# mmaker/c-lwe-snarks

Measured on AMD Instinct MI355X. Metric: snark_proofs_per_sec, higher is better.
Workload: dtype u32 limbs (704-bit integers mod 2^704) + AES-256 bytes; int8 digits on the matrix cores, int32 accumulation (exact)

## Files before the change

c-lwe-snarks_amd/csrc/ctx.hpp:

```cpp
#pragma once
#include <hip/hip_runtime.h>

#include <stdint.h>
#include <string.h>

#include <string>
#include <vector>

#include "aes_dev.hpp"
#include "mfhip.h"
#include "ssp_prg.hpp"

#define HIP_TRY(ctx, expr)                                                        \
  do {                                                                            \
    hipError_t e_ = (expr);                                                       \
    if (e_ != hipSuccess) {                                                       \
      (ctx)->err = std::string(#expr) + ": " + hipGetErrorString(e_);             \
      return MFH_EDEVICE;                                                         \
    }                                                                             \
  } while (0)

struct PolyState;
struct SspInterp;
struct SspRows;
// ... 262 lines not shown
  uint64_t cstride;
  uint32_t bits_row0;
  const uint64_t *add_ct;
  const uint32_t *add_scale;
  uint32_t sa_from1;
};
int eval_rows_multi_io(mfh_ctx *c, uint64_t off, size_t nrows, const uint8_t *d_c8, const MmIo &io, uint32_t nvec, uint32_t coeff_bytes, int accumulate);
int eval_rows_multi_io_set(mfh_ctx *c, uint64_t off, size_t nrows, const uint8_t *d_c8, const MmIo *ios, const uint32_t *nvecs, uint32_t ng,
                           uint32_t coeff_bytes);
struct MmRegion { uint64_t off; const uint8_t *c8; };
int eval_rows_multi_io_regions(mfh_ctx *c, const MmRegion *regs, uint32_t nreg, size_t nrows, const MmIo *ios, const uint32_t *nvecs, uint32_t ng,
                               uint32_t coeff_bytes, int accumulate);
bool mm_image_covers(const mfh_ctx *c, uint64_t off, size_t nrows);
struct MmsPlan {
  uint32_t ng, ngt, ND, nrows, nchunks, rpc, rpad, ntiles, mtiles;
  size_t cd_bytes, part_bytes;
  const uint8_t *img[2];
  int8_t *cd;
  int *part;
};
bool mms_plan(mfh_ctx *c, const MmRegion *regs, uint32_t nreg, size_t nrows, const MmIo *ios, const uint32_t *nvecs, uint32_t ng, uint32_t coeff_bytes,
              MmsPlan &P);
size_t mms_ws_bytes(const MmsPlan &P);
void mms_bind(MmsPlan &P, void *ws);
int mms_digits(mfh_ctx *c, const MmsPlan &P, const MmIo *ios, const uint32_t *nvecs);
int mms_stream(mfh_ctx *c, const MmsPlan &P);
int mms_finish(mfh_ctx *c, const MmsPlan &P, const MmIo *ios, const uint32_t *nvecs, int accumulate);
```

c-lwe-snarks_amd/csrc/evalmm.hip:

```cpp
#include <algorithm>
#include <cstring>

#include "ctx.hpp"

namespace {

using mf::AesKey;

constexpr int CT = 4;
constexpr int SB = 88;
constexpr int VB = 92;
constexpr int MB = CT * SB;
constexpr int MT = MB / 32;
constexpr int RT = 128;
constexpr int TSTRIDE = 384;
constexpr int BLK_PER_ROW = 24;
static_assert(MB % 32 == 0 && CT * VB + 15 <= TSTRIDE, "tile geometry");

typedef int v4i __attribute__((ext_vector_type(4)));
typedef int v16i __attribute__((ext_vector_type(16)));

__device__ __forceinline__ uint32_t coef_at(const MmIo &io, uint32_t v, uint32_t nrows, uint32_t i) {
  if (io.bits) {
    const uint32_t a = io.bits_row0 + i;
// ... 467 lines not shown
constexpr int CH = NQ2 / CG;
struct MmsImages { const v4i *image[16]; };
__device__ __forceinline__ void mms_item(uint32_t xcd, uint32_t slot, uint32_t ngt, uint32_t ngr, uint32_t map, uint32_t &grp, uint32_t &tg) {
  if (map == 0) {
    grp = slot % ngt;
    tg = (slot / ngt) * 8 + xcd;
  } else {
    const uint32_t blk = slot >> 5, i = slot & 31, nreg = ngt / ngr, tpb = 32 / ngr;
    grp = (blk % nreg) * ngr + i % ngr;
    tg = ((blk / nreg) * tpb + i / ngr) * 8 + xcd;
  }
}
__device__ __forceinline__ long long mms_pack_e(const v4i &a) {
  return (long long)a[0] + ((long long)a[1] << 8) + ((long long)a[2] << 16) + ((long long)a[3] << 24);
}
template <int CTRL>
__device__ __forceinline__ long long mms_quad_bcast(long long t) {
  const int lo = __builtin_amdgcn_update_dpp(0, (int)(unsigned int)(unsigned long long)t, CTRL, 0xf, 0xf, false);
  const int hi = __builtin_amdgcn_update_dpp(0, (int)((unsigned long long)t >> 32), CTRL, 0xf, 0xf, false);
  return (long long)(((unsigned long long)(unsigned int)hi << 32) | (unsigned int)lo);
}
__device__ __forceinline__ void mms_store_packed(int *__restrict__ part, uint32_t pk, uint64_t m4 , uint32_t ctile, uint32_t c16,
                                                 const v4i &acc) {
  const long long T = mms_pack_e(acc);
  if (pk == 1) {
    reinterpret_cast<long long *>(part)[m4 * N2 + 16 * ctile + c16] = T;
    return;
  }
  const long long T1 = mms_quad_bcast<0x55>(T), T2 = mms_quad_bcast<0xAA>(T), T3 = mms_quad_bcast<0xFF>(T);
  if (c16 & 3) return;
  const __int128 U = (__int128)T + (__int128)T1 * 256 + (__int128)T2 * 65536 + (__int128)T3 * 16777216;
  const unsigned __int128 u = (unsigned __int128)U;
  reinterpret_cast<uint4 *>(part)[m4 * (N2 / 4) + 4 * ctile + (c16 >> 2)] = uint4{(uint32_t)u, (uint32_t)(u >> 32), (uint32_t)(u >> 64), 0u};
}
__device__ __forceinline__ void mmstream_body(const MmsImages &imgs, uint32_t mtiles, uint32_t KS, uint32_t nrows, uint32_t rows_per_chunk,
                                              const v4i *__restrict__ cdv, int *__restrict__ part, uint32_t grp, uint32_t tg ,
                                              uint32_t chunk, uint64_t cd_stride , uint64_t part_stride , uint32_t pk ) {
  __shared__ v4i bfrag[2][RT2 / 64][NQ2][64];
  const uint32_t tid = threadIdx.x, lane = tid & 63;
  const uint32_t wave = __builtin_amdgcn_readfirstlane(tid >> 6);
  const uint32_t c16 = lane & 15, g4 = lane >> 4;
  const uint32_t rq = wave % RG, ch = wave / RG;
  if (tg * 16 >= mtiles) return;
  const v4i *__restrict__ image = imgs.image[grp];
  cdv += grp * cd_stride;
  part += grp * part_stride;
  const uint32_t mt0 = (tg * RG + rq) * RQ;
  const uint32_t r0 = chunk * rows_per_chunk, r1 = min(nrows, r0 + rows_per_chunk);
  v4i acc[RQ][CH];
#pragma unroll
  for (int t = 0; t < RQ; t++)
#pragma unroll
    for (int q = 0; q < CH; q++) acc[t][q] = v4i{0, 0, 0, 0};
// ... 70 lines not shown
#pragma unroll
      for (int t = 0; t < RQ; t++) a[t][ks] = a_load(t, un1, ks);
#pragma unroll
      for (int i = 0; i < BPK; i++) bnr[ks][i] = b_load(un2, ks, i);
    }
#ifndef MMS_NOSYNC
    __syncthreads();
#endif
    buf ^= 1;
  }
  const uint64_t Mtot = (uint64_t)mtiles * 16;
#ifdef MMS_ACC_ASM
  asm volatile("s_nop 15\n\ts_nop 15" ::: "memory");
#endif
  if (pk) {
#pragma unroll
    for (int t = 0; t < RQ; t++) {
      if (mt0 + t >= mtiles) continue;
      const uint64_t m4 = (uint64_t)chunk * (Mtot / 4) + (uint64_t)(mt0 + t) * 4 + g4;
#pragma unroll
      for (int q = 0; q < CH; q++) mms_store_packed(part, pk, m4, ch * CH + q, c16, acc[t][q]);
    }
    return;
  }
#pragma unroll
  for (int t = 0; t < RQ; t++) {
    if (mt0 + t >= mtiles) continue;
    int *p = part + ((uint64_t)chunk * Mtot + (uint64_t)(mt0 + t) * 16) * N2;
#pragma unroll
    for (int q = 0; q < CH; q++)
#pragma unroll
      for (int e = 0; e < 4; e++) p[(uint64_t)(4 * g4 + e) * N2 + 16 * (ch * CH + q) + c16] = acc[t][q][e];
  }
}

__global__ __launch_bounds__(SW * 64) void k_mmstream(MmsImages imgs, uint32_t mtiles, uint32_t KS, uint32_t nrows, uint32_t rows_per_chunk,
                                                      const v4i *__restrict__ cdv, int *__restrict__ part, uint32_t ngt, uint32_t ngr, uint32_t map,
                                                      uint64_t cd_stride, uint64_t part_stride, uint32_t pk) {
  uint32_t grp, tg;
  mms_item(blockIdx.x & 7, blockIdx.x >> 3, ngt, ngr, map, grp, tg);
  mmstream_body(imgs, mtiles, KS, nrows, rows_per_chunk, cdv, part, grp, tg, blockIdx.y, cd_stride, part_stride, pk);
}
__global__ __launch_bounds__(SW * 64) void k_mmstream1(MmsImages imgs, uint32_t mtiles, uint32_t KS, uint32_t nrows, uint32_t rows_per_chunk,
                                                       const v4i *__restrict__ cdv, int *__restrict__ part, uint32_t pk) {
  mmstream_body(imgs, mtiles, KS, nrows, rows_per_chunk, cdv, part, 0u, blockIdx.x, blockIdx.y, 0, 0, pk);
}
__device__ __forceinline__ void mmstream_persistent(const MmsImages &imgs, uint32_t mtiles, uint32_t KS, uint32_t nrows, uint32_t rows_per_chunk,
                                                    const v4i *__restrict__ cdv, int *__restrict__ part, uint32_t ngt, uint32_t ngr, uint32_t map,
                                                    uint64_t cd_stride, uint64_t part_stride, uint32_t nblk , uint32_t nchunks,
                                                    uint32_t *__restrict__ sync, uint32_t sync_mode, uint32_t spin_max, uint32_t width, uint32_t pk) {
  const uint32_t xcd = blockIdx.x & 7, cu = blockIdx.x >> 3;
  const uint32_t members = sync_mode == 2 ? 32u : (map ? ngr : ngt);
  uint32_t *ctr = sync + xcd * 32 + (sync_mode == 2 ? 0u : cu / members);
  uint32_t k = 0;
  for (uint32_t chunk = 0; chunk < nchunks; chunk++)
    for (uint32_t slot = cu; slot < nblk * 32; slot += width, k++) {
      if (sync_mode && members > 1) {
        if (threadIdx.x == 0) {
          __hip_atomic_fetch_add(ctr, 1u, __ATOMIC_RELAXED, __HIP_MEMORY_SCOPE_AGENT);
          const uint32_t target = (k + 1) * members;
          for (uint32_t spin = 0; spin < spin_max && __hip_atomic_load(ctr, __ATOMIC_RELAXED, __HIP_MEMORY_SCOPE_AGENT) < target; spin++) __builtin_amdgcn_s_sleep(8);
        }
        __syncthreads();
      }
      uint32_t grp, tg;
      mms_item(xcd, slot, ngt, ngr, map, grp, tg);
      mmstream_body(imgs, mtiles, KS, nrows, rows_per_chunk, cdv, part, grp, tg, chunk, cd_stride, part_stride, pk);
    }
}
__global__ __launch_bounds__(SW * 64) void k_mmstream_p(MmsImages imgs, uint32_t mtiles, uint32_t KS, uint32_t nrows, uint32_t rows_per_chunk,
                                                        const v4i *__restrict__ cdv, int *__restrict__ part, uint32_t ngt, uint32_t ngr, uint32_t map,
                                                        uint64_t cd_stride, uint64_t part_stride, uint32_t nblk, uint32_t nchunks,
                                                        uint32_t *__restrict__ sync, uint32_t sync_mode, uint32_t spin_max, uint32_t width, uint32_t pk) {
  mmstream_persistent(imgs, mtiles, KS, nrows, rows_per_chunk, cdv, part, ngt, ngr, map, cd_stride, part_stride, nblk, nchunks, sync, sync_mode, spin_max, width, pk);
}
__global__ __launch_bounds__(SW * 64) void k_mmstream_pb(MmsImages imgs, uint32_t mtiles, uint32_t KS, uint32_t nrows, uint32_t rows_per_chunk,
                                                         const v4i *__restrict__ cdv, int *__restrict__ part, uint32_t ngt, uint32_t ngr, uint32_t map,
                                                         uint64_t cd_stride, uint64_t part_stride, uint32_t nblk, uint32_t nchunks,
                                                         uint32_t *__restrict__ sync, uint32_t sync_mode, uint32_t spin_max, uint32_t width, uint32_t pk) {
  mmstream_persistent(imgs, mtiles, KS, nrows, rows_per_chunk, cdv, part, ngt, ngr, map, cd_stride, part_stride, nblk, nchunks, sync, sync_mode, spin_max, width, pk);
}

constexpr int WSW = 4, WRQ = 4;
__device__ __forceinline__ void mfma_acc(v4i &acc, const v4i &a, const v4i &b) {
  asm volatile("v_mfma_i32_16x16x64_i8 %0, %1, %2, %0" : "+a"(acc) : "v"(a), "v"(b));
}
__device__ __forceinline__ void mmstream_body_w(const MmsImages &imgs, uint32_t mtiles, uint32_t KS, uint32_t nrows, uint32_t rows_per_chunk,
                                                const v4i *__restrict__ cdv, int *__restrict__ part, uint32_t grp, uint32_t tg, uint32_t chunk, uint64_t cd_stride,
                                                uint64_t part_stride) {
  __shared__ v4i bfrag[2][RT2 / 64][NQ2][64];
  const uint32_t tid = threadIdx.x, lane = tid & 63;
  const uint32_t wave = __builtin_amdgcn_readfirstlane(tid >> 6);
  const uint32_t c16 = lane & 15, g4 = lane >> 4;
  if (tg * 16 >= mtiles) return;
  const v4i *__restrict__ image = imgs.image[grp];
// ... 90 lines not shown
                                                         const v4i *__restrict__ cdv, int *__restrict__ part, uint32_t ngt, uint32_t ngr, uint32_t map,
                                                         uint64_t cd_stride, uint64_t part_stride, uint32_t nblk, uint32_t nchunks) {
  const uint32_t xcd = blockIdx.x & 7, cu = blockIdx.x >> 3;
  for (uint32_t k = 0; k < nblk * nchunks; k++) {
    uint32_t grp, tg;
    mms_item(xcd, (k % nblk) * 32 + cu, ngt, ngr, map, grp, tg);
    mmstream_body_w(imgs, mtiles, KS, nrows, rows_per_chunk, cdv, part, grp, tg, k / nblk, cd_stride, part_stride);
  }
}

template <int ND, int KWM ,
          bool PK >
__device__ __forceinline__ void evalmm_finish_body(const int *__restrict__ part, const int64_t *__restrict__ sc, uint32_t nchunks, uint32_t ntiles, uint32_t N,
                                                   uint32_t nvec, uint32_t n, uint32_t nrows, uint32_t ct, uint32_t MBv, uint32_t sby, uint32_t LL,
                                                   const MmIo &io, int accumulate, const int *__restrict__ sa_part, uint32_t sa_col) {
  __shared__ uint32_t sv[KWM][3][64];
  const uint32_t vl = threadIdx.x & 63, lq = threadIdx.x >> 6;
  const uint32_t v = blockIdx.y * 64 + vl, j = blockIdx.x;
  const uint32_t tile = j / ct, jj = j % ct;
  const uint32_t KWv = sby / 4;
  if (v < nvec) {
    int64_t corr[ND];
#pragma unroll
    for (int w = 0; w < ND; w++) corr[w] = 128 * sc[ND * v + w] + 16384ll * nrows;
    if (PK) {
      const uint64_t M4 = (uint64_t)ntiles * MBv / 4;
      unsigned __int128 corrsum = 0;
#pragma unroll
      for (int w = 0; w < ND; w++) corrsum += (unsigned __int128)((uint64_t)corr[w] * 0x01010101ull) << (8 * w);
      for (uint32_t l = lq; l < KWv; l += 4) {
        const uint64_t m4 = ((uint64_t)tile * MBv + jj * sby) / 4 + l;
        __int128 U = 0, SA = 0;
        for (uint32_t ch = 0; ch < nchunks; ch++) {
          const uint64_t at = (uint64_t)ch * M4 + m4;
          if (ND == 4) {
            const uint4 r = reinterpret_cast<const uint4 *>(part)[at * (N / 4) + v], q = reinterpret_cast<const uint4 *>(sa_part)[at * (N / 4) + sa_col / 4];
            U += (__int128)(((unsigned __int128)(uint64_t)(int64_t)(int32_t)r.z << 64) | ((uint64_t)r.y << 32) | r.x);
            SA += (__int128)(((unsigned __int128)(uint64_t)(int64_t)(int32_t)q.z << 64) | ((uint64_t)q.y << 32) | q.x);
          } else {
            U += reinterpret_cast<const long long *>(part)[at * N + v];
            SA += reinterpret_cast<const long long *>(sa_part)[at * N + sa_col];
          }
        }
        const unsigned __int128 val = (unsigned __int128)(U + SA * (__int128)(ND == 4 ? 128ll * 0x01010101ll : 128ll)) + corrsum;
        sv[l][0][vl] = (uint32_t)val;
        sv[l][1][vl] = (uint32_t)(val >> 32);
        sv[l][2][vl] = (uint32_t)(val >> 64);
      }
    } else
    for (uint32_t l = lq; l < KWv; l += 4) {
      unsigned __int128 val = 0;
      int g0[4][ND], sa0[4];
#pragma unroll
      for (int k = 0; k < 4; k++) {
        const int *row = part + ((uint64_t)tile * MBv + (jj * sby + 4 * l + k)) * N;
#pragma unroll
        for (int w = 0; w < ND; w++) g0[k][w] = row[ND * v + w];
        sa0[k] = (sa_part + ((uint64_t)tile * MBv + (jj * sby + 4 * l + k)) * N)[sa_col];
      }
#pragma unroll
      for (int k = 0; k < 4; k++) {
        const uint32_t mm = jj * sby + 4 * l + k;
        int64_t g[ND], sa = sa0[k];
#pragma unroll
        for (int w = 0; w < ND; w++) g[w] = g0[k][w];
        for (uint32_t ch = 1; ch < nchunks; ch++) {
          const int *row = part + (((uint64_t)ch * ntiles + tile) * MBv + mm) * N;
#pragma unroll
          for (int w = 0; w < ND; w++) g[w] += row[ND * v + w];
          sa += (sa_part + (((uint64_t)ch * ntiles + tile) * MBv + mm) * N)[sa_col];
        }
        uint64_t t = 0;
#pragma unroll
        for (int w = 0; w < ND; w++) t += (uint64_t)(g[w] + 128 * sa + corr[w]) << (8 * w);
        val += (unsigned __int128)t << (8 * k);
      }
      sv[l][0][vl] = (uint32_t)val;
      sv[l][1][vl] = (uint32_t)(val >> 32);
      sv[l][2][vl] = (uint32_t)(val >> 64);
    }
  }
  __syncthreads();
  if (lq != 0 || v >= nvec) return;
  uint32_t *out = reinterpret_cast<uint32_t *>((v < io.osplit ? io.out[0] + (uint64_t)v * io.ostride : io.out[1] + (uint64_t)(v - io.osplit) * io.ostride) +
                                               (uint64_t)j * LL);
  const bool wide4 = (LL & 1) == 0 && (io.ostride & 1) == 0 && ((reinterpret_cast<uintptr_t>(io.out[0]) | reinterpret_cast<uintptr_t>(io.out[1])) & 15) == 0;
  uint32_t pend[4] = {0, 0, 0, 0};
  uint64_t carry = 0;
  const uint32_t *actw = io.add_ct ? reinterpret_cast<const uint32_t *>(io.add_ct + (uint64_t)j * LL) : nullptr;
  const uint64_t ax = io.add_ct ? io.add_scale[v] : 0;
  uint64_t acarry = 0;
  for (uint32_t l = 0; l < KWv; l++) {
    uint64_t word = carry + sv[l][0][vl];
    if (l >= 1) word += sv[l - 1][1][vl];
    if (l >= 2) word += sv[l - 2][2][vl];
    if (accumulate) word += out[l];
    if (actw) {
      const uint64_t t = (uint64_t)actw[l] * ax + acarry;
      word += (uint32_t)t;
      acarry = t >> 32;
    }
    carry = word >> 32;
    pend[l & 3] = (uint32_t)word;
    if (wide4 ? (l & 3) == 3 : (l & 1) == 1) {
      if (wide4) *reinterpret_cast<uint4 *>(out + (l & ~3u)) = uint4{pend[0], pend[1], pend[2], pend[3]};
      else *reinterpret_cast<uint2 *>(out + (l & ~1u)) = uint2{pend[(l & 2)], pend[(l & 2) + 1]};
    }
  }
  if (wide4) {
    if (KWv & 3) *reinterpret_cast<uint4 *>(out + (KWv & ~3u)) = uint4{pend[0], (KWv & 3) > 1 ? pend[1] : 0u, (KWv & 3) > 2 ? pend[2] : 0u, 0u};
// ... 16 lines not shown
                                                               int accumulate) {
  const uint32_t g = blockIdx.z, lender = A.io[g].sa_from1 ? A.io[g].sa_from1 - 1 : g;
  evalmm_finish_body<ND, KWM, PK>(part + g * part_stride, A.io[g].sc_zeroed, nchunks, ntiles, N, A.nvec[g], n, nrows, ct, MBv, sby, LL, A.io[g], accumulate,
                                  part + lender * part_stride, ND * A.nvec[lender]);
}

}

extern "C" {

struct WideGeom { uint32_t ct, sby, vby, mt, mbp, LL; };
static WideGeom wide_geom(const mfh_ctx *c) {
  if (c->P.logq == 736) return {W16<736>::CT, W16<736>::SBY, W16<736>::VBY, W16<736>::MT, W16<736>::MBP, W16<736>::LL};
  return {W16<1472>::CT, W16<1472>::SBY, W16<1472>::VBY, W16<1472>::MT, W16<1472>::MBP, W16<1472>::LL};
}

#define FINISH_LAUNCH(kern, ND_, PK_, grid, ...)                                                                         \
  do {                                                                                                                   \
    if ((PK_) && wg.sby / 4 <= 22) hipLaunchKernelGGL((kern<ND_, 22, true>), grid, dim3(256), 0, c->stream, __VA_ARGS__);  \
    else if (PK_) hipLaunchKernelGGL((kern<ND_, 46, true>), grid, dim3(256), 0, c->stream, __VA_ARGS__);                 \
    else if (wg.sby / 4 <= 22) hipLaunchKernelGGL((kern<ND_, 22, false>), grid, dim3(256), 0, c->stream, __VA_ARGS__);   \
    else hipLaunchKernelGGL((kern<ND_, 46, false>), grid, dim3(256), 0, c->stream, __VA_ARGS__);                         \
  } while (0)

int mfh_eval_rows_multi(mfh_ctx *c, uint64_t off, size_t nrows, const uint8_t *d_c8, const uint32_t *d_coeffs, uint32_t nvec, uint32_t coeff_bytes,
                        uint64_t *d_rops, int accumulate) {
  if (!c || !d_rops || !nvec || (nrows && (!d_c8 || !d_coeffs)) || (coeff_bytes != 1 && coeff_bytes != 4)) return MFH_EINVAL;
  const MmIo io = {{d_coeffs, nullptr}, nvec, {d_rops, nullptr}, nvec, (uint64_t)(c->P.n + 1) * wide_geom(c).LL, nullptr, 0, nullptr};
  return eval_rows_multi_io(c, off, nrows, d_c8, io, nvec, coeff_bytes, accumulate);
}
// ... 29 lines not shown
    }
    return MFH_OK;
  }
  const uint32_t ct = wide ? wg.ct : CT, mb = wide ? wg.mbp : CT * SB, rt = wide ? RT2 : RT;
  const uint32_t NT = wide ? NQ2 : (nvec * ND + 1 <= 64 ? 2 : 4), N = wide ? N2 : 32 * NT;
  const uint32_t ntiles = (n + 1 + ct - 1) / ct;
  uint32_t nchunks = (!wide && nrows >= 8 * rt) ? 2 : 1;
  const uint32_t lim = std::max(rt, c->mm_chunk_rows / rt * rt);
  nchunks = std::max<uint32_t>(nchunks, ((uint32_t)nrows + lim - 1) / lim);
  uint32_t rpc = ((uint32_t)nrows + nchunks - 1) / nchunks;
  rpc = (rpc + rt - 1) / rt * rt;
  nchunks = ((uint32_t)nrows + rpc - 1) / rpc;
  const uint32_t rpad = nchunks * rpc;
  const size_t cd_bytes = ((size_t)N * rpad + 255) & ~(size_t)255;
  const size_t sc_bytes = 256 * 8;
  const size_t part_bytes = (size_t)nchunks * ntiles * mb * N * 4;
  int rc = c->mm_ws_sel ? ws2_reserve(c, cd_bytes + sc_bytes + part_bytes) : ws_reserve(c, cd_bytes + sc_bytes + part_bytes);
  if (rc) return rc;
  uint8_t *wsp = (c->mm_ws_sel ? c->ws2 : c->ws).as<uint8_t>();
  int8_t *cd = (int8_t *)wsp;
  int64_t *sc = io.sc_zeroed ? io.sc_zeroed : (int64_t *)(wsp + cd_bytes);
  int *part = (int *)(wsp + cd_bytes + sc_bytes);
  if (!io.sc_zeroed) HIP_TRY(c, hipMemsetAsync(sc, 0, sc_bytes, c->stream));
  if (wide && ND == 4 && !io.bits)
    hipLaunchKernelGGL(k_mm_digits4w, dim3((rpad / 16 + DG4 - 1) / DG4), dim3(256), 0, c->stream, io, nvec, (uint32_t)nrows, rpad, cd, sc);
  else
    hipLaunchKernelGGL(k_mm_digits, dim3((rpad / 16 + DG_RG - 1) / DG_RG), dim3(N), 0, c->stream, io, nvec, ND, (uint32_t)nrows, rpad, NT, wide ? 1 : 0, cd, sc);
  AesKey keyx = c->key;
  for (int i = 56; i < 60; i++) keyx.rk[i] ^= 0x80808080u;
  const uint32_t pk = img_region && c->mm_pack ? ND : 0u;
  {
    Timer t(c, img_region ? 8 : 7, nrows);
    if (img_region) {
      const uint32_t mtiles = ntiles * wg.mt, KS = ((uint32_t)nrows + RT2 - 1) / RT2 * (RT2 / 64);
      MmsImages imgs{};
      imgs.image[0] = (const v4i *)img_region;
      hipLaunchKernelGGL(k_mmstream1, dim3(((mtiles + TPW - 1) / TPW + 7) / 8 * 8, nchunks), dim3(SW * 64), 0, c->stream, imgs,
                         mtiles, KS, (uint32_t)nrows, rpc, (const v4i *)cd, part, pk);
    } else if (wide && q736)
      hipLaunchKernelGGL((k_evalmm16<0, 736>), dim3(ntiles, nchunks), dim3(1024), 0, c->stream, keyx, c->d_t0, off, n, (uint32_t)nrows, rpc, d_c8, cd, part,
                         (uint8_t *)nullptr);
    else if (wide)
      hipLaunchKernelGGL((k_evalmm16<0, 1472>), dim3(ntiles, nchunks), dim3(1024), 0, c->stream, keyx, c->d_t0, off, n, (uint32_t)nrows, rpc, d_c8, cd, part,
                         (uint8_t *)nullptr);
    else if (NT == 2)
      hipLaunchKernelGGL(k_evalmm<2>, dim3(ntiles, nchunks), dim3(1024), 0, c->stream, keyx, c->d_t0, off, n, (uint32_t)nrows, rpc, d_c8, cd, rpad,
                         part);
    else
      hipLaunchKernelGGL(k_evalmm<4>, dim3(ntiles, nchunks), dim3(1024), 0, c->stream, keyx, c->d_t0, off, n, (uint32_t)nrows, rpc, d_c8, cd, rpad,
                         part);
  }
  HIP_TRY(c, hipGetLastError());
  const uint32_t sby = wide ? wg.sby : SB;
  const dim3 fgrid(n + 1, (nvec + 63) / 64);
  if (ND == 4)
    FINISH_LAUNCH(k_evalmm_finish, 4, pk, fgrid, part, sc, nchunks, ntiles, N, nvec, n, (uint32_t)nrows, ct, mb, sby, wg.LL, io, accumulate);
  else
    FINISH_LAUNCH(k_evalmm_finish, 1, pk, fgrid, part, sc, nchunks, ntiles, N, nvec, n, (uint32_t)nrows, ct, mb, sby, wg.LL, io, accumulate);
  HIP_TRY(c, hipGetLastError());
  return MFH_OK;
}

bool mms_plan(mfh_ctx *c, const MmRegion *regs, uint32_t nreg, size_t nrows, const MmIo *ios, const uint32_t *nvecs, uint32_t ng, uint32_t coeff_bytes,
              MmsPlan &P) {
  if (!c || !regs || !ios || !nvecs || !ng || !nreg || nreg > 2 || nreg * ng > 16) return false;
  bool ok = nreg * ng > 1 && c->have_seed && nrows && nrows <= 0xffffffffu - 256;
  for (uint32_t q = 0; q < nreg && ok; q++) {
    P.img[q] = nullptr;
    for (int r = 0; r < 3 && c->mm_image; r++)
      if (c->mm_off[r] == regs[q].off && c->mm_rows[r] == nrows) P.img[q] = c->mm_image + c->mm_base[r];
    ok = P.img[q] != nullptr;
  }
  P.ng = ng;
  P.ngt = nreg * ng;
  for (uint32_t g = 0; g < P.ngt && ok; g++) {
    ok = nvecs[g] && nvecs[g] * coeff_bytes + (ios[g].sa_from1 ? 0 : 1) <= 256 && ios[g].out[0] && ios[g].sc_zeroed && (ios[g].bits || ios[g].coef[0]);
    if (ok && ios[g].sa_from1) {
// ... 2 lines not shown
      for (uint32_t x = 0; x < P.ngt && ok; x++) ok = !ios[x].bits;
    }
  }
  if (!ok) return false;
  const WideGeom wg = wide_geom(c);
  P.ND = coeff_bytes;
  P.nrows = (uint32_t)nrows;
  P.ntiles = (c->P.n + 1 + wg.ct - 1) / wg.ct;
  P.mtiles = P.ntiles * wg.mt;
  const uint32_t lim = std::max<uint32_t>(RT2, c->mm_chunk_rows / RT2 * RT2);
  uint32_t nchunks = ((uint32_t)nrows + lim - 1) / lim;
  P.rpc = (((uint32_t)nrows + nchunks - 1) / nchunks + RT2 - 1) / RT2 * RT2;
  P.nchunks = ((uint32_t)nrows + P.rpc - 1) / P.rpc;
  P.rpad = P.nchunks * P.rpc;
  P.cd_bytes = ((size_t)N2 * P.rpad + 255) & ~(size_t)255;
  P.part_bytes = ((size_t)P.nchunks * P.ntiles * wg.mbp * N2 * 4 + 255) & ~(size_t)255;
  P.cd = nullptr;
  P.part = nullptr;
  return true;
}
size_t mms_ws_bytes(const MmsPlan &P) { return (size_t)P.ngt * (P.cd_bytes + P.part_bytes); }
void mms_bind(MmsPlan &P, void *ws) {
  P.cd = (int8_t *)ws;
  P.part = (int *)((uint8_t *)ws + (size_t)P.ngt * P.cd_bytes);
}
static bool mms_group_args(const MmsPlan &P, const MmIo *ios, const uint32_t *nvecs, MmGroupArgs &A) {
  if (P.ND != 4) return false;
  for (uint32_t g = 0; g < P.ngt; g++) {
    if (ios[g].bits) return false;
    A.io[g] = ios[g];
    A.nvec[g] = nvecs[g];
// ... 6 lines not shown
    hipLaunchKernelGGL(k_mm_digits4w_groups, dim3((P.rpad / 16 + DG4 - 1) / DG4, P.ngt), dim3(256), 0, c->stream, A, P.nrows, P.rpad, P.cd, (uint64_t)P.cd_bytes);
    HIP_TRY(c, hipGetLastError());
    return MFH_OK;
  }
  for (uint32_t g = 0; g < P.ngt; g++) {
    if (P.ND == 4 && !ios[g].bits)
      hipLaunchKernelGGL(k_mm_digits4w, dim3((P.rpad / 16 + DG4 - 1) / DG4), dim3(256), 0, c->stream, ios[g], nvecs[g], P.nrows, P.rpad, P.cd + g * P.cd_bytes,
                         ios[g].sc_zeroed);
    else
      hipLaunchKernelGGL(k_mm_digits, dim3((P.rpad / 16 + DG_RG - 1) / DG_RG), dim3(N2), 0, c->stream, ios[g], nvecs[g], P.ND, P.nrows, P.rpad, (uint32_t)NQ2, 1,
                         P.cd + g * P.cd_bytes, ios[g].sc_zeroed);
  }
  HIP_TRY(c, hipGetLastError());
  return MFH_OK;
}
static bool mms_persistent(const mfh_ctx *c, const MmsPlan &P) {
  return P.ngt > 1 && c->mm_persist && c->ncu == 256 && ((c->mm_map && 32 % P.ng == 0) || 32 % P.ngt == 0);
}
static uint32_t mms_pk(const mfh_ctx *c, const MmsPlan &P) {
  if (!c->mm_pack || (mms_persistent(c, P) && c->mm_wave1)) return 0;
  return P.ND;
}
int mms_stream(mfh_ctx *c, const MmsPlan &P) {
  const uint32_t KS = (P.nrows + RT2 - 1) / RT2 * (RT2 / 64), tgs = (P.mtiles + TPW - 1) / TPW;
  const bool will_persist = mms_persistent(c, P);
  Timer t(c, P.ngt > 1 ? (P.ND == 1 ? 14 : 10) : 8, P.nrows, (uint64_t)P.nrows * P.ngt, will_persist ? 1 : 0);
  MmsImages imgs{};
  for (uint32_t g = 0; g < P.ngt; g++) imgs.image[g] = (const v4i *)P.img[g / P.ng];
  const uint32_t pk = mms_pk(c, P);
  if (P.ngt > 1) {
    const uint32_t tgx = (tgs + 7) / 8;
    const uint32_t map = c->mm_map && 32 % P.ng == 0 ? 1u : 0u;
    const uint32_t slots = map ? (tgx + 32 / P.ng - 1) / (32 / P.ng) * (P.ngt / P.ng) * 32 : tgx * P.ngt;
    const bool persistent = will_persist;
    if (persistent && c->mm_wave1) {
      hipLaunchKernelGGL(k_mmstream_w, dim3(256), dim3(WSW * 64), 0, c->stream, imgs, P.mtiles, KS, P.nrows, P.rpc, (const v4i *)P.cd, P.part, P.ngt, P.ng, map,
                         (uint64_t)(P.cd_bytes / 16), (uint64_t)(P.part_bytes / 4), (slots + 31) / 32, P.nchunks);
    } else if (persistent) {
      if (!c->mm_sync) HIP_TRY(c, hipMalloc(&c->mm_sync, 8 * 32 * sizeof(uint32_t)));
      if (c->mm_sync_mode) HIP_TRY(c, hipMemsetAsync(c->mm_sync, 0, 8 * 32 * sizeof(uint32_t), c->stream));
      const uint32_t width = P.ND == 1 ? 32u : c->mm_width;
      hipLaunchKernelGGL(P.ND == 1 ? k_mmstream_pb : k_mmstream_p, dim3(8 * width), dim3(SW * 64), 0, c->stream, imgs, P.mtiles, KS, P.nrows, P.rpc, (const v4i *)P.cd, P.part, P.ngt, P.ng, map,
                         (uint64_t)(P.cd_bytes / 16), (uint64_t)(P.part_bytes / 4), (slots + 31) / 32, P.nchunks, c->mm_sync, width == 32 ? c->mm_sync_mode : 0u, c->mm_spin, width, pk);
    } else {
      hipLaunchKernelGGL(k_mmstream, dim3(slots * 8, P.nchunks), dim3(SW * 64), 0, c->stream, imgs, P.mtiles, KS, P.nrows, P.rpc, (const v4i *)P.cd, P.part, P.ngt, P.ng,
                         map, (uint64_t)(P.cd_bytes / 16), (uint64_t)(P.part_bytes / 4), pk);
    }
  } else
    hipLaunchKernelGGL(k_mmstream1, dim3((tgs + 7) / 8 * 8, P.nchunks), dim3(SW * 64), 0, c->stream, imgs, P.mtiles, KS, P.nrows, P.rpc, (const v4i *)P.cd, P.part, pk);
  HIP_TRY(c, hipGetLastError());
  return MFH_OK;
}
int mms_finish(mfh_ctx *c, const MmsPlan &P, const MmIo *ios, const uint32_t *nvecs, int accumulate) {
  const WideGeom wg = wide_geom(c);
  const uint32_t n = c->P.n;
  const uint32_t pk = mms_pk(c, P);
  MmGroupArgs A;
  if (mms_group_args(P, ios, nvecs, A)) {
    uint32_t nvmax = 0;
    for (uint32_t g = 0; g < P.ngt; g++) nvmax = std::max(nvmax, nvecs[g]);
    FINISH_LAUNCH(k_evalmm_finish_groups, 4, pk, dim3(n + 1, (nvmax + 63) / 64, P.ngt), P.part, (uint64_t)(P.part_bytes / 4), P.nchunks, P.ntiles, (uint32_t)N2, n, P.nrows,
                  wg.ct, wg.mbp, wg.sby, wg.LL, A, accumulate);
    HIP_TRY(c, hipGetLastError());
    return MFH_OK;
  }
  for (uint32_t g = 0; g < P.ngt; g++) {
    const dim3 fgrid(n + 1, (nvecs[g] + 63) / 64);
    int *pg = P.part + g * (P.part_bytes / 4);
    if (P.ND == 4)
      FINISH_LAUNCH(k_evalmm_finish, 4, pk, fgrid, pg, ios[g].sc_zeroed, P.nchunks, P.ntiles, (uint32_t)N2, nvecs[g], n, P.nrows, wg.ct, wg.mbp, wg.sby, wg.LL, ios[g],
                    accumulate);
// ... 141 lines not shown
```

Before: 13780.

## Store packed matmul partials as per-row-tile carry records

The stream kernel previously wrote one packed 64-bit or 96-bit partial per row per column. It now stages each wave's accumulators in spare shared memory and folds a whole 16-row tile into a single carried record (lo64 plus a high word). This shrinks the partial buffer and the finish kernel's reads and chunk reductions, and the finish kernel changes to decode and recombine those records with a split-half offset for the 736-bit geometry. In exchange it adds wave-level syncs, 128-bit arithmetic in the store path and more complex indexing that must handle tile-boundary coordinate splits correctly.

```diff
diff --git a/c-lwe-snarks_amd/csrc/ctx.hpp b/c-lwe-snarks_amd/csrc/ctx.hpp
--- a/c-lwe-snarks_amd/csrc/ctx.hpp
+++ b/c-lwe-snarks_amd/csrc/ctx.hpp
@@ -300,6 +300,7 @@
 bool mm_image_covers(const mfh_ctx *c, uint64_t off, size_t nrows);
 struct MmsPlan {
   uint32_t ng, ngt, ND, nrows, nchunks, rpc, rpad, ntiles, mtiles;
+  uint32_t pk;
   size_t cd_bytes, part_bytes;
   const uint8_t *img[2];
   int8_t *cd;
diff --git a/c-lwe-snarks_amd/csrc/evalmm.hip b/c-lwe-snarks_amd/csrc/evalmm.hip
--- a/c-lwe-snarks_amd/csrc/evalmm.hip
+++ b/c-lwe-snarks_amd/csrc/evalmm.hip
@@ -505,29 +505,54 @@
 __device__ __forceinline__ long long mms_pack_e(const v4i &a) {
   return (long long)a[0] + ((long long)a[1] << 8) + ((long long)a[2] << 16) + ((long long)a[3] << 24);
 }
-template <int CTRL>
-__device__ __forceinline__ long long mms_quad_bcast(long long t) {
-  const int lo = __builtin_amdgcn_update_dpp(0, (int)(unsigned int)(unsigned long long)t, CTRL, 0xf, 0xf, false);
-  const int hi = __builtin_amdgcn_update_dpp(0, (int)((unsigned long long)t >> 32), CTRL, 0xf, 0xf, false);
-  return (long long)(((unsigned long long)(unsigned int)hi << 32) | (unsigned int)lo);
-}
-__device__ __forceinline__ void mms_store_packed(int *__restrict__ part, uint32_t pk, uint64_t m4 , uint32_t ctile, uint32_t c16,
-                                                 const v4i &acc) {
-  const long long T = mms_pack_e(acc);
-  if (pk == 1) {
-    reinterpret_cast<long long *>(part)[m4 * N2 + 16 * ctile + c16] = T;
-    return;
-  }
-  const long long T1 = mms_quad_bcast<0x55>(T), T2 = mms_quad_bcast<0xAA>(T), T3 = mms_quad_bcast<0xFF>(T);
-  if (c16 & 3) return;
-  const __int128 U = (__int128)T + (__int128)T1 * 256 + (__int128)T2 * 65536 + (__int128)T3 * 16777216;
-  const unsigned __int128 u = (unsigned __int128)U;
-  reinterpret_cast<uint4 *>(part)[m4 * (N2 / 4) + 4 * ctile + (c16 >> 2)] = uint4{(uint32_t)u, (uint32_t)(u >> 32), (uint32_t)(u >> 64), 0u};
+__host__ __device__ constexpr uint32_t trec_count(uint32_t pk) { return pk == 4 ? N2 / 4 : N2; }
+__host__ __device__ constexpr uint32_t trec_bytes(uint32_t pk) { return pk == 4 ? 24u : 20u; }
+__device__ __forceinline__ __int128 trec_sext96(uint32_t a, uint32_t b, uint32_t c) {
+  return (__int128)(((unsigned __int128)(uint64_t)(int64_t)(int32_t)c << 64) | ((uint64_t)b << 32) | a);
+}
+__device__ __forceinline__ void trec_wave_sync() {
+  __builtin_amdgcn_fence(__ATOMIC_RELEASE, "wavefront");
+  __builtin_amdgcn_wave_barrier();
+  __builtin_amdgcn_fence(__ATOMIC_ACQUIRE, "wavefront");
+}
+__device__ __forceinline__ void trec_store(uint8_t *__restrict__ rec, uint32_t pk, bool split, uint32_t r, const __int128 (&X)[4]) {
+  const __int128 two32 = (__int128)1 << 32;
+  const __int128 A = X[0] + X[1] * two32, B = X[2] + X[3] * two32;
+  const uint64_t lo = (uint64_t)A;
+  const unsigned __int128 H = (unsigned __int128)(split ? B : B + (A >> 64));
+  reinterpret_cast<uint4 *>(rec)[r] = uint4{(uint32_t)lo, (uint32_t)(lo >> 32), (uint32_t)H, (uint32_t)(H >> 32)};
+  if (pk == 4) reinterpret_cast<uint2 *>(rec + trec_count(4) * 16)[r] = uint2{(uint32_t)(H >> 64), (uint32_t)(H >> 96)};
+  else reinterpret_cast<uint32_t *>(rec + trec_count(1) * 16)[r] = (uint32_t)(H >> 64);
+}
+template <int CHn>
+__device__ __forceinline__ void mms_store_tile(uint8_t *__restrict__ rec , long long *__restrict__ xch ,
+                                               uint32_t pk, bool split, uint32_t ct0, uint32_t lane, const v4i (&acc)[CHn]) {
+#pragma unroll
+  for (int q = 0; q < CHn; q++) xch[q * 64 + lane] = mms_pack_e(acc[q]);
+  trec_wave_sync();
+  if (pk == 4) {
+    for (uint32_t r = lane; r < CHn * 4; r += 64) {
+      const long long *tp = xch + (r >> 2) * 64 + 4 * (r & 3);
+      __int128 X[4];
+#pragma unroll
+      for (int g = 0; g < 4; g++) X[g] = (__int128)tp[16 * g] + (__int128)tp[16 * g + 1] * 256 + (__int128)tp[16 * g + 2] * 65536 + (__int128)tp[16 * g + 3] * 16777216;
+      trec_store(rec, 4, split, 4 * ct0 + r, X);
+    }
+  } else {
+    for (uint32_t r = lane; r < CHn * 16; r += 64) {
+      const long long *tp = xch + (r >> 4) * 64 + (r & 15);
+      const __int128 X[4] = {tp[0], tp[16], tp[32], tp[48]};
+      trec_store(rec, 1, split, 16 * ct0 + r, X);
+    }
+  }
+  trec_wave_sync();
 }
 __device__ __forceinline__ void mmstream_body(const MmsImages &imgs, uint32_t mtiles, uint32_t KS, uint32_t nrows, uint32_t rows_per_chunk,
                                               const v4i *__restrict__ cdv, int *__restrict__ part, uint32_t grp, uint32_t tg ,
-                                              uint32_t chunk, uint64_t cd_stride , uint64_t part_stride , uint32_t pk ) {
+                                              uint32_t chunk, uint64_t cd_stride , uint64_t part_stride , uint32_t pk ,
+                                              uint32_t ctm ) {
   __shared__ v4i bfrag[2][RT2 / 64][NQ2][64];
+  static_assert(SW * CH * 64 * sizeof(long long) <= sizeof(bfrag[1]), "tile records: every wave parks a row tile's T in its share of the second buffer");
   const uint32_t tid = threadIdx.x, lane = tid & 63;
   const uint32_t wave = __builtin_amdgcn_readfirstlane(tid >> 6);
   const uint32_t c16 = lane & 15, g4 = lane >> 4;
@@ -628,12 +653,14 @@
   asm volatile("s_nop 15\n\ts_nop 15" ::: "memory");
 #endif
   if (pk) {
+    uint32_t ln = lane;
+    asm volatile("" : "+v"(ln));
 #pragma unroll
     for (int t = 0; t < RQ; t++) {
       if (mt0 + t >= mtiles) continue;
-      const uint64_t m4 = (uint64_t)chunk * (Mtot / 4) + (uint64_t)(mt0 + t) * 4 + g4;
-#pragma unroll
-      for (int q = 0; q < CH; q++) mms_store_packed(part, pk, m4, ch * CH + q, c16, acc[t][q]);
+      uint8_t *rec = reinterpret_cast<uint8_t *>(part) + ((uint64_t)chunk * mtiles + mt0 + t) * (trec_count(pk) * trec_bytes(pk));
+      const bool split = ctm && (mt0 + t) % ctm == ctm / 2;
+      mms_store_tile<CH>(rec, reinterpret_cast<long long *>(&bfrag[1][0][0][0]) + wave * (CH * 64), pk, split, ch * CH, ln, acc[t]);
     }
     return;
   }
@@ -650,19 +677,19 @@
 
 __global__ __launch_bounds__(SW * 64) void k_mmstream(MmsImages imgs, uint32_t mtiles, uint32_t KS, uint32_t nrows, uint32_t rows_per_chunk,
                                                       const v4i *__restrict__ cdv, int *__restrict__ part, uint32_t ngt, uint32_t ngr, uint32_t map,
-                                                      uint64_t cd_stride, uint64_t part_stride, uint32_t pk) {
+                                                      uint64_t cd_stride, uint64_t part_stride, uint32_t pk, uint32_t ctm) {
   uint32_t grp, tg;
   mms_item(blockIdx.x & 7, blockIdx.x >> 3, ngt, ngr, map, grp, tg);
-  mmstream_body(imgs, mtiles, KS, nrows, rows_per_chunk, cdv, part, grp, tg, blockIdx.y, cd_stride, part_stride, pk);
+  mmstream_body(imgs, mtiles, KS, nrows, rows_per_chunk, cdv, part, grp, tg, blockIdx.y, cd_stride, part_stride, pk, ctm);
 }
 __global__ __launch_bounds__(SW * 64) void k_mmstream1(MmsImages imgs, uint32_t mtiles, uint32_t KS, uint32_t nrows, uint32_t rows_per_chunk,
-                                                       const v4i *__restrict__ cdv, int *__restrict__ part, uint32_t pk) {
-  mmstream_body(imgs, mtiles, KS, nrows, rows_per_chunk, cdv, part, 0u, blockIdx.x, blockIdx.y, 0, 0, pk);
+                                                       const v4i *__restrict__ cdv, int *__restrict__ part, uint32_t pk, uint32_t ctm) {
+  mmstream_body(imgs, mtiles, KS, nrows, rows_per_chunk, cdv, part, 0u, blockIdx.x, blockIdx.y, 0, 0, pk, ctm);
 }
 __device__ __forceinline__ void mmstream_persistent(const MmsImages &imgs, uint32_t mtiles, uint32_t KS, uint32_t nrows, uint32_t rows_per_chunk,
                                                     const v4i *__restrict__ cdv, int *__restrict__ part, uint32_t ngt, uint32_t ngr, uint32_t map,
                                                     uint64_t cd_stride, uint64_t part_stride, uint32_t nblk , uint32_t nchunks,
-                                                    uint32_t *__restrict__ sync, uint32_t sync_mode, uint32_t spin_max, uint32_t width, uint32_t pk) {
+                                                    uint32_t *__restrict__ sync, uint32_t sync_mode, uint32_t spin_max, uint32_t width, uint32_t pk, uint32_t ctm) {
   const uint32_t xcd = blockIdx.x & 7, cu = blockIdx.x >> 3;
   const uint32_t members = sync_mode == 2 ? 32u : (map ? ngr : ngt);
   uint32_t *ctr = sync + xcd * 32 + (sync_mode == 2 ? 0u : cu / members);
@@ -679,20 +706,20 @@
       }
       uint32_t grp, tg;
       mms_item(xcd, slot, ngt, ngr, map, grp, tg);
-      mmstream_body(imgs, mtiles, KS, nrows, rows_per_chunk, cdv, part, grp, tg, chunk, cd_stride, part_stride, pk);
+      mmstream_body(imgs, mtiles, KS, nrows, rows_per_chunk, cdv, part, grp, tg, chunk, cd_stride, part_stride, pk, ctm);
     }
 }
 __global__ __launch_bounds__(SW * 64) void k_mmstream_p(MmsImages imgs, uint32_t mtiles, uint32_t KS, uint32_t nrows, uint32_t rows_per_chunk,
                                                         const v4i *__restrict__ cdv, int *__restrict__ part, uint32_t ngt, uint32_t ngr, uint32_t map,
                                                         uint64_t cd_stride, uint64_t part_stride, uint32_t nblk, uint32_t nchunks,
-                                                        uint32_t *__restrict__ sync, uint32_t sync_mode, uint32_t spin_max, uint32_t width, uint32_t pk) {
-  mmstream_persistent(imgs, mtiles, KS, nrows, rows_per_chunk, cdv, part, ngt, ngr, map, cd_stride, part_stride, nblk, nchunks, sync, sync_mode, spin_max, width, pk);
+                                                        uint32_t *__restrict__ sync, uint32_t sync_mode, uint32_t spin_max, uint32_t width, uint32_t pk, uint32_t ctm) {
+  mmstream_persistent(imgs, mtiles, KS, nrows, rows_per_chunk, cdv, part, ngt, ngr, map, cd_stride, part_stride, nblk, nchunks, sync, sync_mode, spin_max, width, pk, ctm);
 }
 __global__ __launch_bounds__(SW * 64) void k_mmstream_pb(MmsImages imgs, uint32_t mtiles, uint32_t KS, uint32_t nrows, uint32_t rows_per_chunk,
                                                          const v4i *__restrict__ cdv, int *__restrict__ part, uint32_t ngt, uint32_t ngr, uint32_t map,
                                                          uint64_t cd_stride, uint64_t part_stride, uint32_t nblk, uint32_t nchunks,
-                                                         uint32_t *__restrict__ sync, uint32_t sync_mode, uint32_t spin_max, uint32_t width, uint32_t pk) {
-  mmstream_persistent(imgs, mtiles, KS, nrows, rows_per_chunk, cdv, part, ngt, ngr, map, cd_stride, part_stride, nblk, nchunks, sync, sync_mode, spin_max, width, pk);
+                                                         uint32_t *__restrict__ sync, uint32_t sync_mode, uint32_t spin_max, uint32_t width, uint32_t pk, uint32_t ctm) {
+  mmstream_persistent(imgs, mtiles, KS, nrows, rows_per_chunk, cdv, part, ngt, ngr, map, cd_stride, part_stride, nblk, nchunks, sync, sync_mode, spin_max, width, pk, ctm);
 }
 
 constexpr int WSW = 4, WRQ = 4;
@@ -813,7 +840,8 @@
 __device__ __forceinline__ void evalmm_finish_body(const int *__restrict__ part, const int64_t *__restrict__ sc, uint32_t nchunks, uint32_t ntiles, uint32_t N,
                                                    uint32_t nvec, uint32_t n, uint32_t nrows, uint32_t ct, uint32_t MBv, uint32_t sby, uint32_t LL,
                                                    const MmIo &io, int accumulate, const int *__restrict__ sa_part, uint32_t sa_col) {
-  __shared__ uint32_t sv[KWM][3][64];
+  constexpr int NREC = (KWM + 2 + 3) / 4;
+  __shared__ uint32_t sv[PK ? NREC * 6 : KWM * 3][64];
   const uint32_t vl = threadIdx.x & 63, lq = threadIdx.x >> 6;
   const uint32_t v = blockIdx.y * 64 + vl, j = blockIdx.x;
   const uint32_t tile = j / ct, jj = j % ct;
@@ -823,28 +851,66 @@
 #pragma unroll
     for (int w = 0; w < ND; w++) corr[w] = 128 * sc[ND * v + w] + 16384ll * nrows;
     if (PK) {
-      const uint64_t M4 = (uint64_t)ntiles * MBv / 4;
-      unsigned __int128 corrsum = 0;
-#pragma unroll
-      for (int w = 0; w < ND; w++) corrsum += (unsigned __int128)((uint64_t)corr[w] * 0x01010101ull) << (8 * w);
-      for (uint32_t l = lq; l < KWv; l += 4) {
-        const uint64_t m4 = ((uint64_t)tile * MBv + jj * sby) / 4 + l;
-        __int128 U = 0, SA = 0;
-        for (uint32_t ch = 0; ch < nchunks; ch++) {
-          const uint64_t at = (uint64_t)ch * M4 + m4;
-          if (ND == 4) {
-            const uint4 r = reinterpret_cast<const uint4 *>(part)[at * (N / 4) + v], q = reinterpret_cast<const uint4 *>(sa_part)[at * (N / 4) + sa_col / 4];
-            U += (__int128)(((unsigned __int128)(uint64_t)(int64_t)(int32_t)r.z << 64) | ((uint64_t)r.y << 32) | r.x);
-            SA += (__int128)(((unsigned __int128)(uint64_t)(int64_t)(int32_t)q.z << 64) | ((uint64_t)q.y << 32) | q.x);
-          } else {
-            U += reinterpret_cast<const long long *>(part)[at * N + v];
-            SA += reinterpret_cast<const long long *>(sa_part)[at * N + sa_col];
-          }
-        }
-        const unsigned __int128 val = (unsigned __int128)(U + SA * (__int128)(ND == 4 ? 128ll * 0x01010101ll : 128ll)) + corrsum;
-        sv[l][0][vl] = (uint32_t)val;
-        sv[l][1][vl] = (uint32_t)(val >> 32);
-        sv[l][2][vl] = (uint32_t)(val >> 64);
+      constexpr uint32_t WB = trec_bytes(ND), NR = trec_count(ND);
+      const uint32_t mtc = MBv / 16, s0 = jj * sby, half = (s0 >> 3) & 1, nrec = ((s0 & 15) + sby + 15) / 16;
+      const uint64_t mtiles = (uint64_t)ntiles * mtc, R0 = (uint64_t)tile * mtc + s0 / 16;
+      uint64_t C = 0;
+#pragma unroll
+      for (int w = 0; w < ND; w++) C += (uint64_t)corr[w] << (8 * w);
+      const unsigned __int128 D = (unsigned __int128)C * 0x0101010101010101ull;
+      const uint64_t KSA = ND == 4 ? 128ull * 0x01010101ull : 128ull;
+      const uint32_t sv_ = ND == 4 ? sa_col / 4 : sa_col;
+      struct Rec { uint4 a; uint2 b; };
+      auto load = [&](const int *base, uint32_t ch, uint32_t k, uint32_t i) -> Rec {
+        const uint8_t *rec = reinterpret_cast<const uint8_t *>(base) + ((uint64_t)ch * mtiles + R0 + k) * (NR * WB);
+        Rec x;
+        x.a = reinterpret_cast<const uint4 *>(rec)[i];
+        if (ND == 4) x.b = reinterpret_cast<const uint2 *>(rec + NR * 16)[i];
+        else x.b = uint2{reinterpret_cast<const uint32_t *>(rec + NR * 16)[i], 0u};
+        return x;
+      };
+      auto lo64 = [](const Rec &x) -> uint64_t { return ((uint64_t)x.a.y << 32) | x.a.x; };
+      auto hi128 = [](const Rec &x) -> unsigned __int128 {
+        if (ND == 4) return ((unsigned __int128)(((uint64_t)x.b.y << 32) | x.b.x) << 64) | (((uint64_t)x.a.w << 32) | x.a.z);
+        return (unsigned __int128)trec_sext96(x.a.z, x.a.w, x.b.x);
+      };
+      constexpr int KPT = (NREC + 3) / 4;
+      Rec r0[KPT], q0[KPT];
+#pragma unroll
+      for (int it = 0; it < KPT; it++) {
+        const uint32_t k = lq + 4 * it;
+        if (k < nrec) {
+          r0[it] = load(part, 0, k, v);
+          q0[it] = load(sa_part, 0, k, sv_);
+        }
+      }
+#pragma unroll
+      for (int it = 0; it < KPT; it++) {
+        const uint32_t k = lq + 4 * it;
+        if (k >= nrec) break;
+        unsigned __int128 ulo = lo64(r0[it]), uhi = hi128(r0[it]), alo = lo64(q0[it]), ahi = hi128(q0[it]);
+        for (uint32_t ch = 1; ch < nchunks; ch++) {
+          const Rec r = load(part, ch, k, v), q = load(sa_part, ch, k, sv_);
+          ulo += lo64(r);
+          uhi += hi128(r);
+          alo += lo64(q);
+          ahi += hi128(q);
+        }
+        unsigned __int128 vlo, vhi;
+        if (half && k == 0) {
+          vlo = 0;
+          vhi = uhi + ahi * KSA + D;
+        } else {
+          vlo = ulo + alo * KSA + (uint64_t)D;
+          vhi = uhi + ahi * KSA + D + (D >> 64) + (vlo >> 64);
+        }
+        uint32_t(*o)[64] = &sv[6 * k];
+        o[0][vl] = (uint32_t)vlo;
+        o[1][vl] = (uint32_t)(vlo >> 32);
+        o[2][vl] = (uint32_t)vhi;
+        o[3][vl] = (uint32_t)(vhi >> 32);
+        o[4][vl] = (uint32_t)(vhi >> 64);
+        o[5][vl] = (uint32_t)(vhi >> 96);
       }
     } else
     for (uint32_t l = lq; l < KWv; l += 4) {
@@ -874,9 +940,9 @@
         for (int w = 0; w < ND; w++) t += (uint64_t)(g[w] + 128 * sa + corr[w]) << (8 * w);
         val += (unsigned __int128)t << (8 * k);
       }
-      sv[l][0][vl] = (uint32_t)val;
-      sv[l][1][vl] = (uint32_t)(val >> 32);
-      sv[l][2][vl] = (uint32_t)(val >> 64);
+      sv[3 * l][vl] = (uint32_t)val;
+      sv[3 * l + 1][vl] = (uint32_t)(val >> 32);
+      sv[3 * l + 2][vl] = (uint32_t)(val >> 64);
     }
   }
   __syncthreads();
@@ -889,10 +955,18 @@
   const uint32_t *actw = io.add_ct ? reinterpret_cast<const uint32_t *>(io.add_ct + (uint64_t)j * LL) : nullptr;
   const uint64_t ax = io.add_ct ? io.add_scale[v] : 0;
   uint64_t acarry = 0;
+  const uint32_t hoff = PK ? (((jj * sby) >> 3) & 1) * 2 : 0;
   for (uint32_t l = 0; l < KWv; l++) {
-    uint64_t word = carry + sv[l][0][vl];
-    if (l >= 1) word += sv[l - 1][1][vl];
-    if (l >= 2) word += sv[l - 2][2][vl];
+    uint64_t word = carry;
+    if (PK) {
+      const uint32_t lp = l + hoff, k = lp >> 2, w = lp & 3;
+      word += sv[6 * k + w][vl];
+      if (k && w < 2) word += sv[6 * (k - 1) + 4 + w][vl];
+    } else {
+      word += sv[3 * l][vl];
+      if (l >= 1) word += sv[3 * (l - 1) + 1][vl];
+      if (l >= 2) word += sv[3 * (l - 2) + 2][vl];
+    }
     if (accumulate) word += out[l];
     if (actw) {
       const uint64_t t = (uint64_t)actw[l] * ax + acarry;
@@ -939,6 +1013,13 @@
   if (c->P.logq == 736) return {W16<736>::CT, W16<736>::SBY, W16<736>::VBY, W16<736>::MT, W16<736>::MBP, W16<736>::LL};
   return {W16<1472>::CT, W16<1472>::SBY, W16<1472>::VBY, W16<1472>::MT, W16<1472>::MBP, W16<1472>::LL};
 }
+
+static size_t mm_part_bytes(uint32_t nchunks, uint32_t mtiles, uint32_t N , uint32_t pk) {
+  const size_t per_tile = pk ? (size_t)trec_count(pk) * trec_bytes(pk) : (size_t)16 * N * 4;
+  return ((size_t)nchunks * mtiles * per_tile + 255) & ~(size_t)255;
+}
+static uint32_t mm_split_period(const WideGeom &wg) { return wg.ct == 2 && wg.sby % 16 == 8 ? wg.mt : 0u; }
+static_assert(W16<736>::SBY % 16 == 8 && W16<736>::MT == 2 * (W16<736>::SBY / 16) + 1 && W16<1472>::CT == 1, "tile records: where a coordinate begins inside a row tile");
 
 #define FINISH_LAUNCH(kern, ND_, PK_, grid, ...)                                                                         \
   do {                                                                                                                   \
@@ -998,7 +1079,8 @@
   const uint32_t rpad = nchunks * rpc;
   const size_t cd_bytes = ((size_t)N * rpad + 255) & ~(size_t)255;
   const size_t sc_bytes = 256 * 8;
-  const size_t part_bytes = (size_t)nchunks * ntiles * mb * N * 4;
+  const uint32_t pk = img_region && c->mm_pack ? ND : 0u;
+  const size_t part_bytes = mm_part_bytes(nchunks, ntiles * mb / 16, N, pk);
   int rc = c->mm_ws_sel ? ws2_reserve(c, cd_bytes + sc_bytes + part_bytes) : ws_reserve(c, cd_bytes + sc_bytes + part_bytes);
   if (rc) return rc;
   uint8_t *wsp = (c->mm_ws_sel ? c->ws2 : c->ws).as<uint8_t>();
@@ -1012,7 +1094,6 @@
     hipLaunchKernelGGL(k_mm_digits, dim3((rpad / 16 + DG_RG - 1) / DG_RG), dim3(N), 0, c->stream, io, nvec, ND, (uint32_t)nrows, rpad, NT, wide ? 1 : 0, cd, sc);
   AesKey keyx = c->key;
   for (int i = 56; i < 60; i++) keyx.rk[i] ^= 0x80808080u;
-  const uint32_t pk = img_region && c->mm_pack ? ND : 0u;
   {
     Timer t(c, img_region ? 8 : 7, nrows);
     if (img_region) {
@@ -1020,7 +1101,7 @@
       MmsImages imgs{};
       imgs.image[0] = (const v4i *)img_region;
       hipLaunchKernelGGL(k_mmstream1, dim3(((mtiles + TPW - 1) / TPW + 7) / 8 * 8, nchunks), dim3(SW * 64), 0, c->stream, imgs,
-                         mtiles, KS, (uint32_t)nrows, rpc, (const v4i *)cd, part, pk);
+                         mtiles, KS, (uint32_t)nrows, rpc, (const v4i *)cd, part, pk, mm_split_period(wg));
     } else if (wide && q736)
       hipLaunchKernelGGL((k_evalmm16<0, 736>), dim3(ntiles, nchunks), dim3(1024), 0, c->stream, keyx, c->d_t0, off, n, (uint32_t)nrows, rpc, d_c8, cd, part,
                          (uint8_t *)nullptr);
@@ -1045,6 +1126,9 @@
   return MFH_OK;
 }
 
+static bool mms_persistent(const mfh_ctx *c, const MmsPlan &P) {
+  return P.ngt > 1 && c->mm_persist && c->ncu == 256 && ((c->mm_map && 32 % P.ng == 0) || 32 % P.ngt == 0);
+}
 bool mms_plan(mfh_ctx *c, const MmRegion *regs, uint32_t nreg, size_t nrows, const MmIo *ios, const uint32_t *nvecs, uint32_t ng, uint32_t coeff_bytes,
               MmsPlan &P) {
   if (!c || !regs || !ios || !nvecs || !ng || !nreg || nreg > 2 || nreg * ng > 16) return false;
@@ -1077,7 +1161,8 @@
   P.nchunks = ((uint32_t)nrows + P.rpc - 1) / P.rpc;
   P.rpad = P.nchunks * P.rpc;
   P.cd_bytes = ((size_t)N2 * P.rpad + 255) & ~(size_t)255;
-  P.part_bytes = ((size_t)P.nchunks * P.ntiles * wg.mbp * N2 * 4 + 255) & ~(size_t)255;
+  P.pk = !c->mm_pack || (mms_persistent(c, P) && c->mm_wave1) ? 0u : P.ND;
+  P.part_bytes = mm_part_bytes(P.nchunks, P.mtiles, N2, P.pk);
   P.cd = nullptr;
   P.part = nullptr;
   return true;
@@ -1114,20 +1199,13 @@
   HIP_TRY(c, hipGetLastError());
   return MFH_OK;
 }
-static bool mms_persistent(const mfh_ctx *c, const MmsPlan &P) {
-  return P.ngt > 1 && c->mm_persist && c->ncu == 256 && ((c->mm_map && 32 % P.ng == 0) || 32 % P.ngt == 0);
-}
-static uint32_t mms_pk(const mfh_ctx *c, const MmsPlan &P) {
-  if (!c->mm_pack || (mms_persistent(c, P) && c->mm_wave1)) return 0;
-  return P.ND;
-}
 int mms_stream(mfh_ctx *c, const MmsPlan &P) {
   const uint32_t KS = (P.nrows + RT2 - 1) / RT2 * (RT2 / 64), tgs = (P.mtiles + TPW - 1) / TPW;
   const bool will_persist = mms_persistent(c, P);
   Timer t(c, P.ngt > 1 ? (P.ND == 1 ? 14 : 10) : 8, P.nrows, (uint64_t)P.nrows * P.ngt, will_persist ? 1 : 0);
   MmsImages imgs{};
   for (uint32_t g = 0; g < P.ngt; g++) imgs.image[g] = (const v4i *)P.img[g / P.ng];
-  const uint32_t pk = mms_pk(c, P);
+  const uint32_t pk = P.pk, ctm = mm_split_period(wide_geom(c));
   if (P.ngt > 1) {
     const uint32_t tgx = (tgs + 7) / 8;
     const uint32_t map = c->mm_map && 32 % P.ng == 0 ? 1u : 0u;
@@ -1141,20 +1219,20 @@
       if (c->mm_sync_mode) HIP_TRY(c, hipMemsetAsync(c->mm_sync, 0, 8 * 32 * sizeof(uint32_t), c->stream));
       const uint32_t width = P.ND == 1 ? 32u : c->mm_width;
       hipLaunchKernelGGL(P.ND == 1 ? k_mmstream_pb : k_mmstream_p, dim3(8 * width), dim3(SW * 64), 0, c->stream, imgs, P.mtiles, KS, P.nrows, P.rpc, (const v4i *)P.cd, P.part, P.ngt, P.ng, map,
-                         (uint64_t)(P.cd_bytes / 16), (uint64_t)(P.part_bytes / 4), (slots + 31) / 32, P.nchunks, c->mm_sync, width == 32 ? c->mm_sync_mode : 0u, c->mm_spin, width, pk);
+                         (uint64_t)(P.cd_bytes / 16), (uint64_t)(P.part_bytes / 4), (slots + 31) / 32, P.nchunks, c->mm_sync, width == 32 ? c->mm_sync_mode : 0u, c->mm_spin, width, pk, ctm);
     } else {
       hipLaunchKernelGGL(k_mmstream, dim3(slots * 8, P.nchunks), dim3(SW * 64), 0, c->stream, imgs, P.mtiles, KS, P.nrows, P.rpc, (const v4i *)P.cd, P.part, P.ngt, P.ng,
-                         map, (uint64_t)(P.cd_bytes / 16), (uint64_t)(P.part_bytes / 4), pk);
+                         map, (uint64_t)(P.cd_bytes / 16), (uint64_t)(P.part_bytes / 4), pk, ctm);
     }
   } else
-    hipLaunchKernelGGL(k_mmstream1, dim3((tgs + 7) / 8 * 8, P.nchunks), dim3(SW * 64), 0, c->stream, imgs, P.mtiles, KS, P.nrows, P.rpc, (const v4i *)P.cd, P.part, pk);
+    hipLaunchKernelGGL(k_mmstream1, dim3((tgs + 7) / 8 * 8, P.nchunks), dim3(SW * 64), 0, c->stream, imgs, P.mtiles, KS, P.nrows, P.rpc, (const v4i *)P.cd, P.part, pk, ctm);
   HIP_TRY(c, hipGetLastError());
   return MFH_OK;
 }
 int mms_finish(mfh_ctx *c, const MmsPlan &P, const MmIo *ios, const uint32_t *nvecs, int accumulate) {
   const WideGeom wg = wide_geom(c);
   const uint32_t n = c->P.n;
-  const uint32_t pk = mms_pk(c, P);
+  const uint32_t pk = P.pk;
   MmGroupArgs A;
   if (mms_group_args(P, ios, nvecs, A)) {
     uint32_t nvmax = 0;
```

Result: no change. 13780 (median of 2 runs) (-0.0%).
